# nkargas/Gen2-UHF-RFID-Reader

Measured on AMD Instinct MI355X. Metric: I/Q Msamples/s through matched_filter->gate->tag_decoder (+ EPC decodes/s), 40 kHz FM0, higher is better.
Workload: dtype f32; 1 GPU; configs[1]: batch of 1024 noise-replicas per GPU of the 71-round file_source_test stand-in trace, FM0 40 kHz BLF @ 2 Msps (1076066 raw I/Q samples each, sigma=0.002), generated and resident in HBM; streams_per_gpu=1024, hbm_bytes_traces=8815132672, parallelism=traces sharded per GPU, no collective

## Files before the change

### gen2-uhf-rfid-reader_amd/csrc/rfid_capi.hip

```cpp
#include <hip/hip_runtime.h>

#include <cmath>
#include <ctime>
#include <pthread.h>
#include <cstdio>
#include <cstdlib>
#include <cstring>
#include <deque>
#include <initializer_list>
#include <map>
#include <memory>
#include <new>
#include <vector>

#include "rfid_host_math.h"
#include "rfid_kernels.hpp"
#include "rfid_inventory.hpp"
#include "rfid_tracks.hpp"
#include "rfid_quality.hpp"
#include "rfid_mi355x.h"
#include "rfid_gen2_host.h"
#define LS2_LAUNCH(kernel, gx, gy, block, args) \
  hipLaunchKernelGGL(rfidk::kernel, dim3((unsigned)(gx), (unsigned)(gy)), dim3((unsigned)(block)), 0, ls2_stream, args)
static thread_local hipStream_t ls2_stream = nullptr;
static thread_local unsigned ls2_front_lds = 0;
#define LS2_LAUNCH_FRONT(kernel, gx, gy, block, args) \
  hipLaunchKernelGGL(rfidk::kernel, dim3((unsigned)(gx), (unsigned)(gy)), dim3((unsigned)(block)), ls2_front_lds, ls2_stream, args)
static double g_la_t[20] = {0};
static long g_la_n[20] = {0};
static bool g_la_on = false;
static inline void la_count(int k, double dt) { if (g_la_on) { g_la_t[k] += dt; g_la_n[k]++; } }
static inline double la_now() { struct timespec ts; clock_gettime(CLOCK_MONOTONIC, &ts); return 1e3 * (double)ts.tv_sec + 1e-6 * (double)ts.tv_nsec; }
struct LaTimer { int k; double t0; explicit LaTimer(int kk) : k(kk), t0(g_la_on ? la_now() : 0.0) {} ~LaTimer() { if (g_la_on) la_count(k, la_now() - t0); } };
#include "rfid_ls2_enqueue.hpp"

using namespace rfidk;

namespace {

struct DevBuf {
  void *p = nullptr;
  size_t cap = 0;
};

}

struct RfidKnobs {
  int long_stream = 1;
  int overlap = 1;
  int ls_calibrate = 1;
  int ls_debug = 0;
  int la_profile = 0;
  int front_unfused = 0;
  int front_chunks = 1;
  int fsm_lanes_min = -1;
  int dc_rounds = -1;
  int la_upload_kernel = 1;
  int front_lds_kb = -1;
  int inventory_slots = 0;
};

struct rfid_ctx {
  rfid_params prm;
  RfidKnobs knobs;
  int device = 0;
  hipStream_t stream = nullptr;
  char err[512];
  float t_cand[N_TCAND];

  rfid_reader_state rs;

  void *d_small = nullptr;
  GateState *d_gate1 = nullptr;
  int *d_io = nullptr;
  DevBuf s_in, s_out;
  DevBuf synth_tab;
  DevBuf ls2_ws;
  DevBuf ls2_ws_alt;
  bool ls2_mark_failed = false;
  bool y_touched = false;
  Ls2Ctl *ls2_host = nullptr;
  Ls2Ctl *d_ls2_ctl = nullptr;
  int ls2_P = 0;
  int ls2_rounds[3] = {0, 0, 0};
  bool ls2_generous = false;
  int ls_mode = 1;
  double ls_fixed_ms = 0.45, ls_ns_per_sample = 0.03, seq_ns_per_sample = 10.2;
  bool ls_calibrated = false;
  bool ls_measured = false;
  bool plan_for_stream = false;
  struct StreamIO {
    bool open = false;
    bool failed = false;
    bool ymode = false;
    int dec() const { return ymode ? 1 : DECIM; }
    int hist() const { return ymode ? 0 : 28; }
    int64_t max_chunk = 0, tail_max = 0;
    float2 *d_buf[2] = {nullptr, nullptr};
    rfid_cf32 *h_pin[2] = {nullptr, nullptr};
    hipStream_t copy_stream = nullptr;
    hipEvent_t ev_up[2] = {nullptr, nullptr};
    hipEvent_t ev_free[2] = {nullptr, nullptr};
    int cur = 0;
    bool pending = false;
    int pend_idx = 0;
    int64_t pend_new = 0;
    int64_t tail_len = 0;
    int64_t acc_new = 0;
    hipEvent_t ev_hist = nullptr;
    int64_t raw_base = 0;
    std::vector<rfid_stream_window> out_w;
    std::vector<rfid_decode_result> out_r;
    struct Pass {
      bool active = false;
// ... 77 lines not shown
  rfid_window *d_swin = nullptr;
  int *d_scount = nullptr;
  rfid_decode_result *d_sres = nullptr;
  rfid_scores *d_sscores = nullptr;
  static const int MF_HIST = NTAPS - 1 + DECIM - 1;
  rfid_cf32 mf_hist[MF_HIST];
  int64_t mf_seen = 0;

  int B = 0;
  int B_plan = 0;
  int64_t max_raw = 0, y_stride = 0;
  float2 *d_y = nullptr;
  float2 *y_view = nullptr;
  float2 *y() const { return y_view ? y_view : d_y; }
  GateState *d_gstate = nullptr;
  rfid_window *d_wtab = nullptr, *d_flat = nullptr;
  int wmax = 0, flat_cap = 0;
  int *d_wcount = nullptr, *d_flat_count = nullptr;
  int *d_ticket = nullptr;
  int ticket_flip = 0;
  rfid_decode_result *d_res = nullptr;
  int *d_sum = nullptr;
  const rfid_decode_result *sum_of = nullptr;
  rfid_scores *d_scores = nullptr;
  rfid_stream_stats *d_stats = nullptr;
  const int64_t *d_lens = nullptr;
  int64_t last_n_raw = 0;
  int decode_grid = 0;
  int n_cus = 256;
  hipEvent_t ev[5] = {nullptr, nullptr, nullptr, nullptr, nullptr};
  bool ev_valid[5] = {false, false, false, false, false};
  static const int MAX_CHUNKS = 16;
  hipStream_t stream2 = nullptr;
  hipEvent_t ev_mf[MAX_CHUNKS + 1], ev_gate[2 * MAX_CHUNKS], ev_pass = nullptr, ev_front_end = nullptr;
  struct ResultSet {
    float2 *d_y = nullptr;
    rfid_window *d_wtab = nullptr, *d_flat = nullptr;
    int *d_wcount = nullptr, *d_flat_count = nullptr;
    rfid_decode_result *d_res = nullptr;
    rfid_stream_stats *d_stats = nullptr;
  } alt;
  bool alt_have = false;
  void *plan_blk = nullptr, *alt_blk = nullptr;
  hipEvent_t ev_fe_done = nullptr, ev_tail_done[2] = {nullptr, nullptr};
  bool tail_recorded[2] = {false, false};
  int set_idx = 0;
  void *alt_y_blk = nullptr;
  hipEvent_t ev_y_free[2] = {nullptr, nullptr};
  bool y_recorded[2] = {false, false};
  int y_idx = 0;
  hipStream_t tail_stream = nullptr;
  struct Stage {
    void *blk = nullptr;
    hipEvent_t ev[2] = {nullptr, nullptr};
    bool enqueued = false;
  };
  struct Inventory : Stage {
    int max_tags = 0, slots = 0;
    rfid_tag_entry *d_ent = nullptr, *d_packed = nullptr;
    int *d_counts = nullptr, *d_over = nullptr, *d_off = nullptr, *d_head = nullptr;
    int n_streams = 0;
  } inv;
  struct Tracks : Stage {
    rfid_tag_read *d_reads = nullptr;
    int64_t cap = 0;
    int64_t *d_off = nullptr;
// ... 16 lines not shown
namespace {

void sio_free(rfid_ctx *c);
int sio_process(rfid_ctx *c, int b, int64_t n_new, bool flush);
int sio_submit(rfid_ctx *c, int b, int64_t n_new, bool flush);
int sio_collect(rfid_ctx *c);
void la_free(rfid_ctx *c);
int la_mf_work(rfid_ctx *c, const rfid_cf32 *in, int n_in, rfid_cf32 *out, int out_cap, int *n_produced);
int la_gate_work(rfid_ctx *c, const rfid_cf32 *in, int n_in, rfid_cf32 *out, int out_cap, int *n_consumed, int *n_written);
int la_gate_swallow(rfid_ctx *c, const rfid_cf32 *in, int n_in, rfid_cf32 *out, int out_cap, int *n_consumed, int *n_written);
bool la_decoder_result(rfid_ctx *c, const rfid_cf32 *in, int wlen, int type, rfid_decode_result *r);

int fail(rfid_ctx *c, int code, const char *what, hipError_t e = hipSuccess) {
  if (c) {
    if (e != hipSuccess)
      snprintf(c->err, sizeof(c->err), "%s: %s", what, hipGetErrorString(e));
    else
      snprintf(c->err, sizeof(c->err), "%s", what);
  }
  return code;
}

struct KnobEntry { const char *name, *env; int RfidKnobs::*field; int lo, hi; };
const KnobEntry g_knob_table[] = {
  {"long_stream", "RFID_LONG_STREAM", &RfidKnobs::long_stream, 0, 2},
  {"overlap", "RFID_OVERLAP", &RfidKnobs::overlap, 0, 2},
  {"ls_calibrate", "RFID_LS_CALIBRATE", &RfidKnobs::ls_calibrate, 0, 1},
  {"ls_debug", "RFID_LS_DEBUG", &RfidKnobs::ls_debug, 0, 1},
  {"la_profile", "RFID_LA_PROFILE", &RfidKnobs::la_profile, 0, 1},
  {"front_unfused", "RFID_FRONT_UNFUSED", &RfidKnobs::front_unfused, 0, 1},
  {"front_chunks", "RFID_FRONT_CHUNKS", &RfidKnobs::front_chunks, 1, rfid_ctx::MAX_CHUNKS},
  {"fsm_lanes_min", "RFID_LS2_FSM_LANES_MIN", &RfidKnobs::fsm_lanes_min, -1, 1 << 30},
  {"dc_rounds", "RFID_LS2_DC_ROUNDS", &RfidKnobs::dc_rounds, -1, 64},
  {"la_upload_kernel", "RFID_LA_UPLOAD_KERNEL", &RfidKnobs::la_upload_kernel, 0, 1},
  {"front_lds_kb", "RFID_LS_FRONT_LDS_KB", &RfidKnobs::front_lds_kb, -1, 64},
  {"inventory_slots", "RFID_INVENTORY_SLOTS", &RfidKnobs::inventory_slots, 0, 1024},
};
int clamp_int(long v, int lo, int hi) { return (int)(v < lo ? lo : (v > hi ? hi : v)); }
void knobs_from_env(RfidKnobs &k) {
  for (const KnobEntry &e : g_knob_table) {
    const char *v = getenv(e.env);
    if (!v || !*v) continue;
    char *end = nullptr;
    const long x = strtol(v, &end, 10);
    if (end == v) continue;
    k.*(e.field) = clamp_int(x, e.lo, e.hi);
  }
}

#define HIPCHK(c, call)                                                     \
  do {                                                                      \
    hipError_t e__ = (call);                                                \
    if (e__ != hipSuccess) return fail((c), RFID_ERR_HIP, #call, e__);      \
  } while (0)

#define HIPCHK_T(c, call)                                                   \
  do {                                                                      \
    hipError_t e__ = (call);                                                \
    if (e__ != hipSuccess) { (c)->y_touched = true; return fail((c), RFID_ERR_HIP, #call, e__); } \
  } while (0)

int grow(rfid_ctx *c, DevBuf &b, size_t bytes) {
  if (bytes <= b.cap) return RFID_OK;
  if (b.p) HIPCHK(c, hipFree(b.p));
  b.p = nullptr;
  b.cap = 0;
  size_t want = bytes < 4096 ? 4096 : bytes;
  HIPCHK(c, hipMalloc(&b.p, want));
// ... 179 lines not shown
    const double t_ls = c->ls_fixed_ms + 1e-6 * c->ls_ns_per_sample * (double)B * (double)n_dec;
    if (pass == 0 && !c->ls_calibrated && t_ls > 0.33 * t_seq && t_ls < 3.0 * t_seq) { ls_calibrate_lazily(c); continue; }
    return t_ls < 0.9 * t_seq;
  }
  return false;
}
bool ls_applicable(rfid_ctx *c, int B, int64_t n_dec) {
  if (c->ls_mode == 0 || B > 4096) return false;
  if (ls2_geometry(B, n_dec).P == 0) return false;
  return c->ls_mode == 2 || ls_pays_off(c, B, n_dec);
}
bool ls_may_apply(const rfid_ctx *c, int B, int64_t n_dec) {
  if (c->ls_mode == 0 || B > 4096) return false;
  if (ls2_geometry(B, n_dec).P == 0) return false;
  const double t_seq = 1e-6 * c->seq_ns_per_sample * (double)n_dec * (double)((B + 1023) / 1024);
  const double t_ls = c->ls_fixed_ms + 1e-6 * c->ls_ns_per_sample * (double)B * (double)n_dec;
  return c->ls_mode == 2 || t_ls < 3.0 * t_seq;
}
size_t ls_workspace_bytes(int B, int64_t n_dec, int64_t y_stride, int wmax) {
  const Ls2Geometry g = ls2_geometry(B, n_dec);
  return g.P ? ls2_layout(g, B, y_stride, wmax).total : 0;
}

int ls_calibrate(rfid_ctx *c);
void ls_note_last_pass(rfid_ctx *c);

struct LsOpts {
  bool carry = false;
  bool hold_last = false;
  bool force = false;
  bool ahead = false;
  const void *raw = nullptr; int64_t raw_stride = 0;
};
void ls_note_last_pass(rfid_ctx *c) {
  if (!c->d_ls2_ctl || !c->ls2_host) return;
  if (hipStreamQuery(c->stream) == hipSuccess) {
    const Ls2Ctl &k = *c->ls2_host;
    if (!c->ls2_generous && k.fail == 0 && k.ok == 0 && k.n_pieces > 0) c->ls2_generous = true;
  }
  (void)hipGetLastError();
}
int ls_enqueue(rfid_ctx *c, int64_t n_dec, const LsOpts &opt, int *enqueued) {
  *enqueued = 0;
  c->d_ls2_ctl = nullptr;
  const Ls2Geometry geo = ls2_geometry(c->B, n_dec);
  if (geo.P == 0 || c->B > 65535) return RFID_OK;
  const Ls2Layout L = ls2_layout(geo, c->B, c->y_stride, c->wmax);
  const bool ahead = opt.ahead && opt.raw && c->ls2_ws.cap >= L.total && c->ls2_ws_alt.cap >= L.total;
  if (opt.ahead && !ahead) return RFID_OK;
  if (L.total > c->ls2_ws.cap) {
    if (c->ls2_ws.p) { (void)hipFree(c->ls2_ws.p); c->ls2_ws.p = nullptr; c->ls2_ws.cap = 0; }
    if (hipMalloc(&c->ls2_ws.p, L.total) != hipSuccess) { (void)hipGetLastError(); c->ls2_ws.p = nullptr; return RFID_OK; }
    c->ls2_ws.cap = L.total;
  }
  if (!c->ls2_host) {
    if (hipHostMalloc((void **)&c->ls2_host, sizeof(Ls2Ctl) + 64, hipHostMallocDefault) != hipSuccess) {
      (void)hipGetLastError(); c->ls2_host = nullptr; return RFID_OK;
    }
    memset(c->ls2_host, 0, sizeof(Ls2Ctl) + 64);
  }
  Ls2Args a;
  memset(&a, 0, sizeof(a));
  a.y = c->y(); a.y_stride = c->y_stride; a.lens = c->d_lens; a.n_dec = n_dec; a.n_streams = c->B;
  if (ahead) std::swap(c->ls2_ws, c->ls2_ws_alt);
  ls2_bind(a, (char *)c->ls2_ws.p, L, geo);
  a.wtab = c->d_wtab; a.wmax = c->wmax; a.wcount = c->d_wcount; a.flat = c->d_flat; a.flat_count = c->d_flat_count; a.flat_cap = c->flat_cap;
  a.carry = opt.carry ? c->d_gstate : nullptr; a.carry_out = opt.carry ? c->d_gstate : nullptr;
  a.hold_last = opt.hold_last ? 1 : 0; a.force = opt.force ? 1 : 0;
  if (opt.raw) {
    a.fused = 1;
    a.raw = (const float2 *)opt.raw; a.raw_stride = opt.raw_stride;
    a.raw_vec_ok = ((opt.raw_stride & 1) == 0 && (((uintptr_t)opt.raw) & 15) == 0) ? 1 : 0;
    a.y_w = c->d_y;
  }
  ls2_stream = ahead ? c->stream2 : c->stream;
  {
    const int kb = (c->knobs.front_lds_kb >= 0) ? c->knobs.front_lds_kb : ((geo.NS >= 32768) ? 10 : 0);
    ls2_front_lds = (unsigned)kb * 1024u;
  }
  a.keep_flat_count = ahead ? 1 : 0;
  {
    static const int lanes_min_default = ls2_fsm_lanes_min();
    ls2_fsm_lanes_min() = (c->knobs.fsm_lanes_min >= 0) ? c->knobs.fsm_lanes_min : lanes_min_default;
  }
  auto mark = [](void *p, int pt) {
    rfid_ctx *cc = (rfid_ctx *)p;
    if (pt == 2) {
      if (ls2_stream == cc->stream2) {
        if (hipEventRecord(cc->ev_fe_done, cc->stream2) != hipSuccess || hipStreamWaitEvent(cc->stream, cc->ev_fe_done, 0) != hipSuccess ||
            hipMemsetAsync(cc->d_flat_count, 0, 2 * sizeof(int), cc->stream) != hipSuccess) cc->ls2_mark_failed = true;
        ls2_stream = cc->stream;
      }
      return;
    }
  };
  c->ls2_mark_failed = false;
  ls2_enqueue(a, true, c->ls2_rounds, c->ls2_generous, c->knobs.dc_rounds, ahead ? +mark : nullptr, c);
  ls2_stream = c->stream;
  HIPCHK(c, hipGetLastError());
  if (c->ls2_mark_failed) return fail(c, RFID_ERR_HIP, "long-stream front end: stream hand-over");
  HIPCHK(c, hipMemcpyAsync(c->ls2_host, a.ctl, sizeof(Ls2Ctl) + sizeof(int), hipMemcpyDeviceToHost, c->stream));
  c->d_ls2_ctl = a.ctl;
  c->ls2_P = geo.P;
  *enqueued = 1;
  if (c->knobs.ls_debug) {
    HIPCHK(c, hipStreamSynchronize(c->stream));
    const Ls2Ctl &k = *c->ls2_host;
    fprintf(stderr, "[ls2] pieces %d P %d fail %d ok %d | avg:", k.n_pieces, geo.P, k.fail, k.ok);
    for (int r = 0; r <= c->ls2_rounds[0]; ++r) fprintf(stderr, " %d/%d", k.avg_count[r], k.avg_list[r]);
    fprintf(stderr, " | fsm:");
    for (int r = 0; r <= c->ls2_rounds[1]; ++r) fprintf(stderr, " %d", k.fsm_count[r]);
    fprintf(stderr, " | dc:");
    for (int r = 0; r <= c->ls2_rounds[2]; ++r) fprintf(stderr, " %d", k.dc_count[r]);
    fprintf(stderr, " | units %d windows %d\n", k.n_units, k.n_windows);
    std::vector<Ls2AvgRun> ar((size_t)geo.NS);
    std::vector<int> aT((size_t)geo.NS);
    std::vector<Ls2Piece> pc((size_t)geo.NS);
    HIPCHK(c, hipMemcpy(ar.data(), a.arun, sizeof(Ls2AvgRun) * ar.size(), hipMemcpyDeviceToHost));
    HIPCHK(c, hipMemcpy(aT.data(), a.aT, sizeof(int) * aT.size(), hipMemcpyDeviceToHost));
    HIPCHK(c, hipMemcpy(pc.data(), a.piece, sizeof(Ls2Piece) * pc.size(), hipMemcpyDeviceToHost));
    long hist_m[8] = {0}, hist_d[8] = {0};
    int shown = 0;
    {
      long hist_len[6] = {0}; int max_len = 0; long n_wide = 0, n_over = 0;
      for (int i = 0; i < geo.NS; ++i) {
        const int len = pc[(size_t)i].len;
        if (len <= 0) continue;
        if (len > max_len) max_len = len;
        const int q = (int)(4.0 * len / geo.P);
        hist_len[q < 2 ? 0 : (q < 4 ? 1 : (q < 6 ? 2 : (q < 8 ? 3 : (q < 16 ? 4 : 5))))]++;
        if (ar[(size_t)i].wide & 2) n_wide++;
        if (ar[(size_t)i].wide & 4) n_over++;
      }
      fprintf(stderr, "[ls2] piece lengths in P (< 0.5, < 1, < 1.5, < 2, < 4, more): %ld %ld %ld %ld %ld %ld, longest %d; last run wide: %ld, exact end put in: %ld\n",
// ... 72 lines not shown
    return RFID_OK;
  }
  hipEvent_t e0 = nullptr, e1 = nullptr;
  bool ok = hipEventCreate(&e0) == hipSuccess && hipEventCreate(&e1) == hipSuccess;
  double t_seq[2] = {0, 0}, t_ls[2] = {0, 0};
  for (int k = 0; k < 2 && ok; ++k) {
    int64_t n = 0;
    const int B = k ? B_big : 1;
    ok = rfid_synth_gen2(c, &p, slots.data(), k ? n_big : n_big / 4, d_base, stride, 0.0f, 77u, 0, &n) == RFID_OK && n == L[k];
    ok = ok && rfid_synth_replicas(c, d_base, L[k], d_many, stride, B, 0.003f, 78u, 0) == RFID_OK;
    ok = ok && rfid_batch_plan(c, B, L[k]) == RFID_OK;
    for (int mode = 0; mode <= 2 && ok; mode += 2) {
      c->ls_mode = mode;
      float best = 1e30f;
      for (int rep = 0; rep < 3 && ok; ++rep) {
        ok = hipEventRecord(e0, c->stream) == hipSuccess && rfid_batch_process(c, d_many, stride, L[k], nullptr, 0) == RFID_OK &&
             hipEventRecord(e1, c->stream) == hipSuccess && hipStreamSynchronize(c->stream) == hipSuccess;
        float ms = 0.0f;
        ok = ok && hipEventElapsedTime(&ms, e0, e1) == hipSuccess;
        if (rep > 0 && ms < best) best = ms;
      }
      if (mode == 2 && ok) ok = c->d_ls2_ctl != nullptr && c->ls2_host->ok != 0;
      (mode ? t_ls : t_seq)[k] = best;
    }
  }
  c->ls_mode = saved_mode;
  if (e0) (void)hipEventDestroy(e0);
  if (e1) (void)hipEventDestroy(e1);
  (void)hipStreamSynchronize(c->stream);
  (void)hipFree(d_base);
  (void)hipFree(d_many);
  free_plan(c);
  c->d_ls2_ctl = nullptr;
  if (!ok) { (void)hipGetLastError(); return RFID_OK; }
  const double n0 = (double)(L[0] / DECIM), n1 = (double)(L[1] / DECIM), N1 = n1 * B_big;
  const double slope = (t_ls[1] - t_ls[0]) / (N1 - n0);
  const double fixed = t_ls[0] - slope * n0;
  if (slope > 0.0 && fixed > 0.0 && t_seq[1] > 0.0) {
    c->ls_ns_per_sample = 1.25 * slope * 1e6;
    c->ls_fixed_ms = fixed;
    c->seq_ns_per_sample = t_seq[1] / n1 * 1e6;
    c->ls_measured = true;
  }
  c->ls_calibrated = true;
  if (c->knobs.ls_debug)
    fprintf(stderr, "[ls2] calibration: fused %.3f / %.3f ms, long-stream %.3f / %.3f ms for 1 x %.0f / %d x %.0f samples -> %.2f ns/sample of the longest trace vs %.3f ms + %.4f ns/sample of all\n",
            t_seq[0], t_seq[1], t_ls[0], t_ls[1], n0, B_big, n1, c->seq_ns_per_sample, c->ls_fixed_ms, c->ls_ns_per_sample);
  return RFID_OK;
}

struct LsCalCache { bool done = false, ok = false; double fixed_ms = 0, ns_all = 0, ns_seq = 0; };
LsCalCache g_ls_cal[64];
pthread_mutex_t g_ls_cal_mu = PTHREAD_MUTEX_INITIALIZER;
void ls_calibrate_lazily(rfid_ctx *c) {
  c->ls_calibrated = true;
  if (!c->knobs.ls_calibrate || c->device < 0 || c->device >= 64) return;
  pthread_mutex_lock(&g_ls_cal_mu);
  LsCalCache &k = g_ls_cal[c->device];
  if (!k.done) {
    k.done = true;
    rfid_ctx *t = nullptr;
    if (rfid_ctx_create(&c->prm, c->device, &t) == RFID_OK && t) {
      t->ls_calibrated = true;
      t->ls_mode = 1;
      if (ls_calibrate(t) == RFID_OK && t->ls_measured) {
        k.ok = true; k.fixed_ms = t->ls_fixed_ms; k.ns_all = t->ls_ns_per_sample; k.ns_seq = t->seq_ns_per_sample;
// ... 51 lines not shown
    pthread_mutex_lock(&prop_mu);
    if (!dev_info[device].known) {
      hipDeviceProp_t prop;
      if (hipGetDeviceProperties(&prop, device) == hipSuccess) {
        dev_info[device].known = true;
        dev_info[device].gfx950 = strncmp(prop.gcnArchName, "gfx950", 6) == 0;
        dev_info[device].cus = prop.multiProcessorCount;
      }
    }
    is_gfx950 = dev_info[device].known && dev_info[device].gfx950;
    pthread_mutex_unlock(&prop_mu);
  }
  if (!is_gfx950) return RFID_ERR_NO_DEVICE;
  rfid_ctx *c = new (std::nothrow) rfid_ctx();
  if (c) c->n_cus = dev_info[device].cus;
  if (!c) return RFID_ERR_CAPACITY;
  c->prm = *p;
  c->device = device;
  c->err[0] = 0;
  compute_t_cand(c->t_cand, p->sample_rate);
  knobs_from_env(c->knobs);
  if (c->knobs.la_profile) g_la_on = true;
  c->ls_mode = c->knobs.long_stream;
  init_reader_state(c);
  memset(c->mf_hist, 0, sizeof(c->mf_hist));
  int rc = RFID_OK;
  do {
    if (hipSetDevice(device) != hipSuccess) { rc = RFID_ERR_NO_DEVICE; break; }
    if (hipStreamCreateWithFlags(&c->stream, hipStreamNonBlocking) != hipSuccess) { rc = RFID_ERR_HIP; break; }
    for (int i = 0; i < 5; ++i)
      if (hipEventCreate(&c->ev[i]) != hipSuccess) { rc = RFID_ERR_HIP; break; }
    if (rc) break;
    if (hipStreamCreateWithFlags(&c->stream2, hipStreamNonBlocking) != hipSuccess) { rc = RFID_ERR_HIP; break; }
    for (int i = 0; i <= rfid_ctx::MAX_CHUNKS; ++i) c->ev_mf[i] = nullptr;
    for (int i = 0; i < 2 * rfid_ctx::MAX_CHUNKS; ++i) c->ev_gate[i] = nullptr;
    if (!rc && (hipEventCreate(&c->ev_pass) != hipSuccess || hipEventCreate(&c->ev_front_end) != hipSuccess ||
                hipEventCreateWithFlags(&c->ev_fe_done, hipEventDisableTiming) != hipSuccess ||
                hipEventCreateWithFlags(&c->ev_tail_done[0], hipEventDisableTiming) != hipSuccess ||
                hipEventCreateWithFlags(&c->ev_tail_done[1], hipEventDisableTiming) != hipSuccess ||
                hipEventCreateWithFlags(&c->ev_y_free[0], hipEventDisableTiming) != hipSuccess ||
                hipEventCreateWithFlags(&c->ev_y_free[1], hipEventDisableTiming) != hipSuccess))
      rc = RFID_ERR_HIP;
    if (rc) break;
    {
      char *blk = nullptr;
      const size_t slot = 256, n_slots = 4 + 1 + 1 + 1 + 1 + 1 + 1;
      if (hipMalloc((void **)&blk, slot * n_slots) != hipSuccess || hipMemset(blk, 0, slot * n_slots) != hipSuccess) { rc = RFID_ERR_HIP; c->d_small = blk; break; }
      static_assert(sizeof(GateState) <= 4 * 256 && sizeof(rfid_scores) <= 256 && sizeof(rfid_decode_result) <= 256, "slots");
      c->d_small = blk;
      c->d_gate1 = (GateState *)blk;
      c->d_io = (int *)(blk + 4 * slot);
      c->d_swin = (rfid_window *)(blk + 5 * slot);
      c->d_scount = (int *)(blk + 6 * slot);
      c->d_ticket = (int *)(blk + 7 * slot);
      c->d_sres = (rfid_decode_result *)(blk + 8 * slot);
      c->d_sscores = (rfid_scores *)(blk + 9 * slot);
    }
  } while (0);
  if (rc != RFID_OK) { rfid_ctx_destroy(c); return rc; }
  *out = c;
  return RFID_OK;
}

int rfid_ctx_destroy(rfid_ctx *c) {
  if (!c) return RFID_ERR_INVALID;
  if (c->knobs.la_profile && (g_la_n[0] || g_la_n[1]))
    fprintf(stderr, "[la] mf_work %ld calls %.2f ms (upload queued %.2f, the call's filter enqueued %.2f, wait for its outputs %.2f, passes submitted from here %.2f) | "
            "gate_work %ld calls %.2f ms | decoder_work %ld calls %.2f ms | reader_work_tx %ld calls %.2f ms | lookahead_enable %.2f ms | "
            "%ld passes: collected %.2f ms (waiting for the device %.2f, fetching windows %.2f), submitted %.2f ms (the pass's filter %.2f, front end's launch list %.2f, "
            "decoder %.2f, packet of results %.2f)\n",
            g_la_n[0], g_la_t[0], g_la_t[4], g_la_t[5], g_la_t[8], g_la_t[6], g_la_n[1], g_la_t[1], g_la_n[2], g_la_t[2], g_la_n[3], g_la_t[3], g_la_t[9],
            g_la_n[10], g_la_t[10], g_la_t[7], g_la_t[12], g_la_t[11], g_la_t[14], g_la_t[13], g_la_t[15], g_la_t[16]);
  (void)hipSetDevice(c->device);
  if (c->stream) (void)hipStreamSynchronize(c->stream);
  la_free(c);
  sio_free(c);
  free_plan(c);
  void *ptrs[] = {c->d_small, c->s_in.p, c->s_out.p, c->synth_tab.p, c->ls2_ws.p, c->ls2_ws_alt.p};
  for (void *p : ptrs)
    if (p) (void)hipFree(p);
  if (c->ls2_host) (void)hipHostFree(c->ls2_host);
  for (int i = 0; i < 5; ++i)
    if (c->ev[i]) (void)hipEventDestroy(c->ev[i]);
  for (rfid_ctx::Stage *st : {(rfid_ctx::Stage *)&c->inv, (rfid_ctx::Stage *)&c->trk, (rfid_ctx::Stage *)&c->qual})
    for (int i = 0; i < 2; ++i)
      if (st->ev[i]) (void)hipEventDestroy(st->ev[i]);
  if (c->stream2) {
    (void)hipStreamSynchronize(c->stream2);
    for (int i = 0; i <= rfid_ctx::MAX_CHUNKS; ++i)
      if (c->ev_mf[i]) (void)hipEventDestroy(c->ev_mf[i]);
    for (int i = 0; i < 2 * rfid_ctx::MAX_CHUNKS; ++i)
      if (c->ev_gate[i]) (void)hipEventDestroy(c->ev_gate[i]);
    if (c->ev_pass) (void)hipEventDestroy(c->ev_pass);
    if (c->ev_front_end) (void)hipEventDestroy(c->ev_front_end);
    if (c->ev_fe_done) (void)hipEventDestroy(c->ev_fe_done);
    for (int i = 0; i < 2; ++i) {
      if (c->ev_tail_done[i]) (void)hipEventDestroy(c->ev_tail_done[i]);
      if (c->ev_y_free[i]) (void)hipEventDestroy(c->ev_y_free[i]);
    }
    (void)hipStreamDestroy(c->stream2);
  }
  if (c->stream) (void)hipStreamDestroy(c->stream);
  delete c;
  return RFID_OK;
}

int rfid_ctx_reset(rfid_ctx *c) {
  if (!c) return RFID_ERR_INVALID;
  HIPCHK(c, hipSetDevice(c->device));
  init_reader_state(c);
  memset(c->mf_hist, 0, sizeof(c->mf_hist));
  c->mf_seen = 0;
  if (c->la.on) { la_free(c); sio_free(c); }
  HIPCHK(c, hipMemsetAsync(c->d_gate1, 0, sizeof(GateState), c->stream));
  HIPCHK(c, hipStreamSynchronize(c->stream));
  return RFID_OK;
}

void *rfid_ctx_stream(rfid_ctx *c) { return c ? (void *)c->stream : nullptr; }

int rfid_get_state(const rfid_ctx *c, rfid_reader_state *out) {
  if (!c || !out) return RFID_ERR_INVALID;
  *out = c->rs;
  return RFID_OK;
}

int rfid_print_results(const rfid_ctx *c, char *buf, int cap, int *len) {
  if (!c || !buf || cap <= 0) return RFID_ERR_INVALID;
  const rfid_reader_state &rs = c->rs;
  int n = 0;
  n += snprintf(buf + n, cap - n, "\n --------------------------\n");
  n += snprintf(buf + n, cap - n, "| Number of queries/queryreps sent : %d\n", rs.n_queries_sent - 1);
  n += snprintf(buf + n, cap - n, "| Current Inventory round : %d\n", rs.cur_inventory_round);
  n += snprintf(buf + n, cap - n, " --------------------------\n");
// ... 155 lines not shown
    e = hipMemset(c->d_wcount, 0, sz_c + sz_fc);
  }
  if (e != hipSuccess) {
    (void)hipGetLastError();
    free_plan(c);
    return fail(c, RFID_ERR_HIP, "rfid_batch_plan: workspace allocation", e);
  }
  c->B = c->B_plan = n_streams;
  if (wide_traces(c)) {
    if (hipMalloc((void **)&c->d_sum, sizeof(int) * ((size_t)c->flat_cap + 4)) != hipSuccess) { (void)hipGetLastError(); c->d_sum = nullptr; }
  }
  {
    const size_t need = sizeof(float2) * (size_t)c->y_stride * n_streams + (sizeof(rfid_window) * 3 + sizeof(rfid_decode_result)) * (size_t)c->flat_cap +
                        sizeof(rfid_stream_stats) * (size_t)n_streams;
    size_t free_b = 0, total_b = 0;
    if (c->knobs.overlap >= 2 && n_streams >= 64 && hipMemGetInfo(&free_b, &total_b) == hipSuccess && need < free_b / 8) {
      hipError_t e2 = hipMalloc(&c->alt_blk, sz_set);
      if (e2 == hipSuccess) {
        bind_set((char *)c->alt_blk, c->alt.d_y, c->alt.d_wtab, c->alt.d_flat, c->alt.d_wcount, c->alt.d_flat_count, c->alt.d_res, c->alt.d_stats);
        e2 = hipMemset(c->alt.d_wcount, 0, sz_c + sz_fc);
      }
      if (e2 == hipSuccess) c->alt_have = true;
      else {
        (void)hipGetLastError();
        if (c->alt_blk) (void)hipFree(c->alt_blk);
        c->alt_blk = nullptr;
        c->alt = rfid_ctx::ResultSet();
      }
    }
  }
  if (ls_may_apply(c, n_streams, n_dec)) {
    {
      size_t free_b = 0, total_b = 0;
      if (!c->alt_have && !c->plan_for_stream && c->knobs.overlap != 0 && sz_y >= ((size_t)16 << 20) && hipMemGetInfo(&free_b, &total_b) == hipSuccess && sz_y < free_b / 8) {
        if (hipMalloc(&c->alt_y_blk, sz_y) == hipSuccess) c->alt.d_y = (float2 *)c->alt_y_blk;
        else { (void)hipGetLastError(); c->alt_y_blk = nullptr; }
      }
    }
    const size_t need = ls_workspace_bytes(n_streams, n_dec, c->y_stride, c->wmax);
    if (need > c->ls2_ws.cap) {
      if (c->ls2_ws.p) (void)hipFree(c->ls2_ws.p);
      c->ls2_ws.p = nullptr; c->ls2_ws.cap = 0;
      if (hipMalloc(&c->ls2_ws.p, need) == hipSuccess) c->ls2_ws.cap = need;
      else { (void)hipGetLastError(); c->ls2_ws.p = nullptr; }
    }
    if (c->alt.d_y && !c->alt_have && (c->knobs.overlap != 0) && c->ls2_ws.p && need > c->ls2_ws_alt.cap) {
      size_t free_b = 0, total_b = 0;
      if (c->ls2_ws_alt.p) (void)hipFree(c->ls2_ws_alt.p);
      c->ls2_ws_alt.p = nullptr; c->ls2_ws_alt.cap = 0;
      if (hipMemGetInfo(&free_b, &total_b) == hipSuccess && need < free_b / 8) {
        if (hipMalloc(&c->ls2_ws_alt.p, need) == hipSuccess) c->ls2_ws_alt.cap = need;
        else { (void)hipGetLastError(); c->ls2_ws_alt.p = nullptr; }
      }
    }
  }
  c->decode_grid = c->n_cus * 8;
  for (int i = 0; i < 5; ++i) c->ev_valid[i] = false;
  return RFID_OK;
}

int rfid_batch_set_streams(rfid_ctx *c, int n_streams) {
  if (!c || n_streams <= 0) return RFID_ERR_INVALID;
  if (!c->B_plan) return RFID_ERR_STATE;
  if (n_streams > c->B_plan) return RFID_ERR_CAPACITY;
  c->B = n_streams;
  return RFID_OK;
}
// ... 330 lines not shown
  *n = nrows;
  if (nrows > cap) return fail(c, RFID_ERR_CAPACITY, "rfid_batch_get_window_quality: cap is smaller than the number of EPC windows");
  const int64_t take = (cap < q.rows) ? cap : q.rows;
  if (take > 0) {
    HIPCHK(c, hipMemcpyAsync(out, q.d_table + (size_t)stream * (size_t)q.rows, sizeof(rfid_read_quality) * (size_t)take, hipMemcpyDeviceToHost, c->stream));
    HIPCHK(c, hipStreamSynchronize(c->stream));
  }
  return RFID_OK;
}

int rfid_batch_quality_ms(rfid_ctx *c, float *ms) {
  if (!c || !ms) return RFID_ERR_INVALID;
  return stage_ms(c, c->qual, ms);
}

int rfid_batch_process(rfid_ctx *c, const void *d_raw, int64_t raw_stride, int64_t n_raw, const void *d_lens,
                       int want_scores) {
  if (!c || !d_raw || n_raw < 0 || raw_stride < n_raw) return RFID_ERR_INVALID;
  if (!c->B) return RFID_ERR_STATE;
  if (n_raw > c->max_raw) return RFID_ERR_CAPACITY;
  ls_note_last_pass(c);
  const int64_t n_out = n_raw / DECIM;
  const int64_t tiles = (n_out + MF_TILE - 1) / MF_TILE;
  const int nch = c->knobs.front_chunks;
  if (nch < 2 && ls_applicable(c, c->B, n_out)) {
    HIPCHK(c, hipSetDevice(c->device));
    { int rj = join_tails(c); if (rj) return rj; }
    int rc;
    if (raw_stride >= 2) {
      c->d_lens = (const int64_t *)d_lens;
      c->last_n_raw = n_raw;
      c->n_chunks_last = 0;
      const bool ahead = c->alt.d_y != nullptr && c->ls2_ws_alt.p != nullptr && !c->alt_have && (c->knobs.overlap != 0);
      if (ahead) {
        std::swap(c->d_y, c->alt.d_y);
        c->y_idx ^= 1;
        if (c->y_touched) {
          HIPCHK_T(c, hipEventRecord(c->ev_pass, c->stream));
          HIPCHK_T(c, hipStreamWaitEvent(c->stream2, c->ev_pass, 0));
          c->y_touched = false;
        }
        if (c->y_recorded[c->y_idx]) {
          HIPCHK_T(c, hipStreamWaitEvent(c->stream2, c->ev_y_free[c->y_idx], 0));
          c->y_recorded[c->y_idx] = false;
        }
      }
      HIPCHK_T(c, hipEventRecord(c->ev[0], c->stream));
      HIPCHK_T(c, hipEventRecord(c->ev[1], c->stream));
      c->ev_valid[0] = c->ev_valid[1] = true;
      int enq = 0;
      LsOpts lo;
      lo.raw = d_raw; lo.raw_stride = raw_stride; lo.ahead = ahead;
      if ((rc = ls_enqueue(c, n_out, lo, &enq))) { c->y_touched = true; return rc; }
      if (!enq && ahead) {
        std::swap(c->d_y, c->alt.d_y); c->y_idx ^= 1;
        c->y_touched = true;
        lo.ahead = false;
        if ((rc = ls_enqueue(c, n_out, lo, &enq))) { c->y_touched = true; return rc; }
      }
      const bool ahead_now = ahead && lo.ahead;
      if (enq) {
        c->fused_last = 2;
        MfFallbackArgs f;
        f.m.x = (const float2 *)d_raw; f.m.x_stride = raw_stride; f.m.n_raw = n_raw; f.m.lens = c->d_lens;
        f.m.n_out = n_out; f.m.in_off = -(NTAPS - 1);
        f.m.vec_ok = ((raw_stride & 1) == 0 && (((uintptr_t)d_raw) & 15) == 0) ? 1 : 0;
        f.m.y = c->d_y; f.m.y_stride = c->y_stride; f.m.tile0 = 0; f.m.stream0 = 0;
        f.skip_if = &c->d_ls2_ctl->ok; f.n_tiles = tiles;
        const int64_t gx = (tiles < 4096) ? tiles : 4096;
        for (int s0 = 0; s0 < c->B && gx > 0; s0 += 65535) {
          f.m.stream0 = s0;
          const int ns = (c->B - s0 < 65535) ? (c->B - s0) : 65535;
          hipLaunchKernelGGL(mf_fallback_kernel, dim3((unsigned)gx, (unsigned)ns), dim3(MF_THREADS), 0, c->stream, f);
          HIPCHK_T(c, hipGetLastError());
        }
        if ((rc = rfid_batch_gate_impl(c, &c->d_ls2_ctl->ok)) || (rc = rfid_batch_decode(c, want_scores)) || (rc = rfid_batch_stats(c))) { c->y_touched = true; return rc; }
        if (ahead_now) {
          HIPCHK_T(c, hipEventRecord(c->ev_y_free[c->y_idx], c->stream));
          c->y_recorded[c->y_idx] = true;
        } else {
          c->y_touched = true;
        }
        return RFID_OK;
      }
    }
    c->y_touched = true;
    if ((rc = batch_mf_on(c, c->stream, d_raw, raw_stride, n_raw, d_lens))) return rc;
    int enq = 0;
    LsOpts lo;
    if ((rc = ls_enqueue(c, n_out, lo, &enq))) return rc;
// ... 142 lines not shown
int rfid_ctx_get_knob(const rfid_ctx *c, const char *name, int *value) {
  if (!c || !name || !value) return RFID_ERR_INVALID;
  for (const KnobEntry &e : g_knob_table)
    if (strcmp(name, e.name) == 0) { *value = (e.field == &RfidKnobs::long_stream) ? c->ls_mode : c->knobs.*(e.field); return RFID_OK; }
  return RFID_ERR_INVALID;
}

int rfid_batch_ls_report(const rfid_ctx *c, rfid_ls_report *out) {
  if (!c || !out) return RFID_ERR_INVALID;
  memset(out, 0, sizeof(*out));
  if (!c->d_ls2_ctl || !c->ls2_host) return RFID_OK;
  (void)hipSetDevice(c->device);
  if (hipStreamSynchronize(c->stream) != hipSuccess) return RFID_ERR_HIP;
  const Ls2Ctl &k = *c->ls2_host;
  const int ra = c->ls2_rounds[0], rf = c->ls2_rounds[1], rd = c->ls2_rounds[2];
  out->pieces = k.n_pieces;
  out->units = k.n_units;
  out->chunk = c->ls2_P;
  out->avg_rounds = k.avg_rounds; out->avg_reruns = k.avg_reruns;
  out->fsm_rounds = k.fsm_rounds;
  out->dc_rounds = k.dc_rounds; out->dc_reruns = k.dc_reruns;
  for (int r = 0; r <= rf; ++r) out->cuts_dropped += k.fsm_count[r];
  out->windows = k.n_windows;
  out->dc_finished = k.dc_finished;
  out->verified = (k.ok != 0) ? 1 : 0;
  out->gave_up = out->verified ? 0 : (k.fail ? k.fail : (k.avg_count[ra] ? 2 : (k.fsm_count[rf] ? 3 : (k.dc_count[rd] ? 4 : 5))));
  return RFID_OK;
}

int rfid_batch_sync(rfid_ctx *c) {
  if (!c) return RFID_ERR_INVALID;
  HIPCHK(c, hipSetDevice(c->device));
  HIPCHK(c, hipStreamSynchronize(c->stream2));
  HIPCHK(c, hipStreamSynchronize(c->stream));
  return RFID_OK;
}

int rfid_batch_timing_get(rfid_ctx *c, rfid_batch_timing *out) {
  if (!c || !out) return RFID_ERR_INVALID;
  HIPCHK(c, hipSetDevice(c->device));
  HIPCHK(c, hipStreamSynchronize(c->stream2));
  HIPCHK(c, hipStreamSynchronize(c->stream));
  float ms[4] = {0, 0, 0, 0};
  float front = 0.0f;
  if (c->n_chunks_last > 0) {
    for (int k = 0; k < c->n_chunks_last; ++k) {
      float t = 0.0f;
      HIPCHK(c, hipEventElapsedTime(&t, c->ev_mf[k], c->ev_mf[k + 1]));
      ms[0] += t;
      HIPCHK(c, hipEventElapsedTime(&t, c->ev_gate[2 * k], c->ev_gate[2 * k + 1]));
      ms[1] += t;
    }
    HIPCHK(c, hipEventElapsedTime(&front, c->ev_mf[0], c->ev_front_end));
    for (int i = 2; i < 4; ++i)
      if (c->ev_valid[i] && c->ev_valid[i + 1]) HIPCHK(c, hipEventElapsedTime(&ms[i], c->ev[i], c->ev[i + 1]));
    out->total_ms = front + ms[2] + ms[3];
  } else {
    for (int i = 0; i < 4; ++i)
      if (c->ev_valid[i] && c->ev_valid[i + 1]) HIPCHK(c, hipEventElapsedTime(&ms[i], c->ev[i], c->ev[i + 1]));
    out->total_ms = ms[0] + ms[1] + ms[2] + ms[3];
  }
  out->mf_ms = ms[0]; out->gate_ms = ms[1]; out->decode_ms = ms[2]; out->stats_ms = ms[3];
  out->front_ms = (c->n_chunks_last > 0) ? front : (ms[0] + ms[1]);
  out->front_chunks = (c->n_chunks_last > 0) ? c->n_chunks_last : 1;
  out->decode_launches = 1;
  out->fused_front = c->fused_last;
  out->reserved_ = 0;
  return RFID_OK;
}

int rfid_batch_get_stats(rfid_ctx *c, rfid_stream_stats *out, int n_streams) {
  if (!c || !out || n_streams <= 0) return RFID_ERR_INVALID;
  if (!c->B) return RFID_ERR_STATE;
  if (n_streams > c->B) n_streams = c->B;
// ... 513 lines not shown
```

### gen2-uhf-rfid-reader_amd/csrc/rfid_ls2_enqueue.hpp

```cpp
#pragma once
#include <stddef.h>
#ifndef LS2_FIN_WPB
#define LS2_FIN_WPB 1
#endif
#ifndef LS2_LAUNCH_FRONT
#define LS2_LAUNCH_FRONT LS2_LAUNCH
#endif
#include <stdint.h>

namespace rfidk {

constexpr int LS2_TARGET_PIECES = 131072;
constexpr int LS2_MIN_PIECE = 512;

struct Ls2Geometry {
  int P = 0, max_b = 0, NS = 0;
  int Pc = 0, max_bc = 0;
  int64_t vstride = 0, cstride = 0, wb_stride = 0;
  int n1 = 0, n2 = 0;
};
inline Ls2Geometry ls2_geometry(int n_streams, int64_t n_dec, int min_piece = LS2_MIN_PIECE, int target = LS2_TARGET_PIECES) {
  Ls2Geometry g;
  if (n_streams <= 0 || n_dec < 2 * (int64_t)LS2_FINE * min_piece) return g;
  int64_t P = ((int64_t)n_streams * n_dec + target - 1) / target;
// ... 154 lines not shown
  } else {
    LS2_LAUNCH(ls2_pieces_kernel, (NS + 255) / 256, 1, 256, a);
  }
  auto rerun_grid = [&](int round, int most) { const int g = (round == 1) ? most : most / 2; return (NS < g) ? NS : g; };
  auto chain_g = [](int slots) { const int per = ls2_chain_slots(); int g = (slots + per - 1) / per; return g < 1 ? 1 : (g > LS2_CHAIN_GMAX ? LS2_CHAIN_GMAX : g); };
  const int g_avg = chain_g(a.max_b), g_seq = chain_g(a.max_bc);
  if (!fused) LS2_LAUNCH(ls2_avg_first_kernel, 8 * ((NS + 7) / 8), 1, 64, a);
  a.chain_g = g_avg; a.stamp++;
  LS2_LAUNCH(ls2_avg_chain_kernel, g_avg, B, LS2_CHAIN_THREADS, a);
  for (int r = 1; r <= a.avg_rounds; ++r) {
    a.round = r;
    LS2_LAUNCH(ls2_avg_rerun_kernel, rerun_grid(r, 32768), 1, 64, a);
    a.stamp++;
    LS2_LAUNCH(ls2_avg_chain_kernel, g_avg, B, LS2_CHAIN_THREADS, a);
  }
  for (int r = 0; r <= a.fsm_rounds; ++r) {
    a.round = r;
    if (NH >= ls2_fsm_lanes_min()) LS2_LAUNCH(ls2_fsm_lanes_kernel, (NH + LS2_FSM_LANES - 1) / LS2_FSM_LANES, 1, 64, U(a));
    else LS2_LAUNCH(ls2_fsm_kernel, NH, 1, 64, U(a));
    LS2_LAUNCH(ls2_fsm_chain_kernel, (NH + 255) / 256, 1, 256, U(a));
  }
  {
    const int N1 = B * a.dcb_n1, N2 = B * a.dcb_n2;
    for (int r = 0; r <= a.dc_rounds; ++r) {
      a.round = r;
      LS2_LAUNCH(ls2_dcb_run_kernel, (r <= 3 || NH < 4096) ? NH : 4096, 1, 64, U(a));
      LS2_LAUNCH(ls2_dcb_up1_kernel, N1, 1, 64, U(a));
      if (a.dcb_top == 2) LS2_LAUNCH(ls2_dcb_up2_kernel, N2, 1, 64, U(a));
      LS2_LAUNCH(ls2_dcb_top_kernel, B, 1, 64, U(a));
      if (a.dcb_top == 2) LS2_LAUNCH(ls2_dcb_down2_kernel, N2, 1, 64, U(a));
      LS2_LAUNCH(ls2_dcb_down1_kernel, N1, 1, 64, U(a));
    }
    a.round = 0;
    {
      LS2_LAUNCH(ls2_dcb_incr_kernel, NH, 1, 64, U(a));
      LS2_LAUNCH(ls2_dcb_finish_kernel<LS2_FIN_WPB>, ls2_fin_waves(B) / LS2_FIN_WPB, B, 64 * LS2_FIN_WPB, U(a));
    }
  }
  a.round = 0;
  a.stamp++;
  a.chain_g = g_seq;
  LS2_LAUNCH(ls2_seq_kernel, g_seq, B, LS2_CHAIN_THREADS, U(a));
  LS2_LAUNCH(ls2_assemble_kernel, NH, 1, 64, U(a));
  if (a.carry_out) LS2_LAUNCH(ls2_carry_kernel, B, 1, 64, U(a));
  if (rounds_out) { rounds_out[0] = a.avg_rounds; rounds_out[1] = a.fsm_rounds; rounds_out[2] = a.dc_rounds; }
}
#endif

}
```

Baseline: 394,900 Msamples/s.

## Add optional second lane stream and multi-slot host control buffers for long-stream overlap

```diff
diff --git a/gen2-uhf-rfid-reader_amd/csrc/rfid_capi.hip b/gen2-uhf-rfid-reader_amd/csrc/rfid_capi.hip
--- a/gen2-uhf-rfid-reader_amd/csrc/rfid_capi.hip
+++ b/gen2-uhf-rfid-reader_amd/csrc/rfid_capi.hip
@@ -55,8 +55,10 @@
   int front_chunks = 1;
   int fsm_lanes_min = -1;
   int dc_rounds = -1;
+  int ls2_alt_min_kb = 16384;
   int la_upload_kernel = 1;
   int front_lds_kb = -1;
+  int ls2_lanes = 1;
   int inventory_slots = 0;
 };
 
@@ -80,6 +82,12 @@
   bool ls2_mark_failed = false;
   bool y_touched = false;
   Ls2Ctl *ls2_host = nullptr;
+  static const int LS2_HOST_SLOTS = 4;
+  static const size_t LS2_HOST_STRIDE = (sizeof(Ls2Ctl) + 64 + 255) & ~(size_t)255;
+  char *ls2_host_blk = nullptr;
+  hipEvent_t ev_ctl[LS2_HOST_SLOTS] = {nullptr, nullptr, nullptr, nullptr};
+  bool ctl_pending[LS2_HOST_SLOTS] = {false, false, false, false};
+  int ctl_slot = 0;
   Ls2Ctl *d_ls2_ctl = nullptr;
   int ls2_P = 0;
   int ls2_rounds[3] = {0, 0, 0};
@@ -223,6 +231,8 @@
   bool ev_valid[5] = {false, false, false, false, false};
   static const int MAX_CHUNKS = 16;
   hipStream_t stream2 = nullptr;
+  hipStream_t stream3 = nullptr;
+  hipEvent_t ev_lane_done[2] = {nullptr, nullptr};
   hipEvent_t ev_mf[MAX_CHUNKS + 1], ev_gate[2 * MAX_CHUNKS], ev_pass = nullptr, ev_front_end = nullptr;
   struct ResultSet {
     float2 *d_y = nullptr;
@@ -305,8 +315,10 @@
   {"front_chunks", "RFID_FRONT_CHUNKS", &RfidKnobs::front_chunks, 1, rfid_ctx::MAX_CHUNKS},
   {"fsm_lanes_min", "RFID_LS2_FSM_LANES_MIN", &RfidKnobs::fsm_lanes_min, -1, 1 << 30},
   {"dc_rounds", "RFID_LS2_DC_ROUNDS", &RfidKnobs::dc_rounds, -1, 64},
+  {"ls2_alt_min_kb", "RFID_LS2_ALT_MIN_KB", &RfidKnobs::ls2_alt_min_kb, 0, 1 << 30},
   {"la_upload_kernel", "RFID_LA_UPLOAD_KERNEL", &RfidKnobs::la_upload_kernel, 0, 1},
   {"front_lds_kb", "RFID_LS_FRONT_LDS_KB", &RfidKnobs::front_lds_kb, -1, 64},
+  {"ls2_lanes", "RFID_LS2_LANES", &RfidKnobs::ls2_lanes, 1, 2},
   {"inventory_slots", "RFID_INVENTORY_SLOTS", &RfidKnobs::inventory_slots, 0, 1024},
 };
 int clamp_int(long v, int lo, int hi) { return (int)(v < lo ? lo : (v > hi ? hi : v)); }
@@ -552,14 +564,23 @@
   bool ahead = false;
   const void *raw = nullptr; int64_t raw_stride = 0;
 };
+void ls_note_slot(rfid_ctx *c, int i) {
+  const Ls2Ctl &k = *(const Ls2Ctl *)(c->ls2_host_blk + (size_t)i * rfid_ctx::LS2_HOST_STRIDE);
+  if (!c->ls2_generous && k.fail == 0 && k.ok == 0 && k.n_pieces > 0) c->ls2_generous = true;
+  c->ctl_pending[i] = false;
+}
 void ls_note_last_pass(rfid_ctx *c) {
-  if (!c->d_ls2_ctl || !c->ls2_host) return;
+  if (!c->ls2_host_blk) return;
+  bool any = false;
+  for (int i = 0; i < rfid_ctx::LS2_HOST_SLOTS; ++i) any = any || c->ctl_pending[i];
+  if (!any) return;
   if (hipStreamQuery(c->stream) == hipSuccess) {
-    const Ls2Ctl &k = *c->ls2_host;
-    if (!c->ls2_generous && k.fail == 0 && k.ok == 0 && k.n_pieces > 0) c->ls2_generous = true;
+    for (int i = 0; i < rfid_ctx::LS2_HOST_SLOTS; ++i)
+      if (c->ctl_pending[i]) ls_note_slot(c, i);
   }
   (void)hipGetLastError();
 }
+hipStream_t ls2_lane_stream(const rfid_ctx *c) { return (c->knobs.ls2_lanes >= 2 && c->y_idx == 1) ? c->stream3 : c->stream2; }
 int ls_enqueue(rfid_ctx *c, int64_t n_dec, const LsOpts &opt, int *enqueued) {
   *enqueued = 0;
   c->d_ls2_ctl = nullptr;
@@ -573,11 +594,18 @@
     if (hipMalloc(&c->ls2_ws.p, L.total) != hipSuccess) { (void)hipGetLastError(); c->ls2_ws.p = nullptr; return RFID_OK; }
     c->ls2_ws.cap = L.total;
   }
-  if (!c->ls2_host) {
-    if (hipHostMalloc((void **)&c->ls2_host, sizeof(Ls2Ctl) + 64, hipHostMallocDefault) != hipSuccess) {
-      (void)hipGetLastError(); c->ls2_host = nullptr; return RFID_OK;
-    }
-    memset(c->ls2_host, 0, sizeof(Ls2Ctl) + 64);
+  if (!c->ls2_host_blk) {
+    const size_t bytes = rfid_ctx::LS2_HOST_STRIDE * rfid_ctx::LS2_HOST_SLOTS;
+    if (hipHostMalloc((void **)&c->ls2_host_blk, bytes, hipHostMallocDefault) != hipSuccess) {
+      (void)hipGetLastError(); c->ls2_host_blk = nullptr; return RFID_OK;
+    }
+    memset(c->ls2_host_blk, 0, bytes);
+    c->ls2_host = (Ls2Ctl *)c->ls2_host_blk;
+  }
+  const int ctl_slot = c->ctl_slot;
+  if (c->ctl_pending[ctl_slot]) {
+    HIPCHK(c, hipEventSynchronize(c->ev_ctl[ctl_slot]));
+    ls_note_slot(c, ctl_slot);
   }
   Ls2Args a;
   memset(&a, 0, sizeof(a));
@@ -593,7 +621,7 @@
     a.raw_vec_ok = ((opt.raw_stride & 1) == 0 && (((uintptr_t)opt.raw) & 15) == 0) ? 1 : 0;
     a.y_w = c->d_y;
   }
-  ls2_stream = ahead ? c->stream2 : c->stream;
+  ls2_stream = ahead ? ls2_lane_stream(c) : c->stream;
   {
     const int kb = (c->knobs.front_lds_kb >= 0) ? c->knobs.front_lds_kb : ((geo.NS >= 32768) ? 10 : 0);
     ls2_front_lds = (unsigned)kb * 1024u;
@@ -605,13 +633,11 @@
   }
   auto mark = [](void *p, int pt) {
     rfid_ctx *cc = (rfid_ctx *)p;
-    if (pt == 2) {
-      if (ls2_stream == cc->stream2) {
-        if (hipEventRecord(cc->ev_fe_done, cc->stream2) != hipSuccess || hipStreamWaitEvent(cc->stream, cc->ev_fe_done, 0) != hipSuccess ||
-            hipMemsetAsync(cc->d_flat_count, 0, 2 * sizeof(int), cc->stream) != hipSuccess) cc->ls2_mark_failed = true;
-        ls2_stream = cc->stream;
-      }
-      return;
+    if (pt == (cc->knobs.ls2_lanes >= 2 ? 3 : 2) && ls2_stream != cc->stream) {
+      hipEvent_t done = cc->ev_lane_done[ls2_stream == cc->stream3 ? 1 : 0];
+      if (hipEventRecord(done, ls2_stream) != hipSuccess || hipStreamWaitEvent(cc->stream, done, 0) != hipSuccess ||
+          hipMemsetAsync(cc->d_flat_count, 0, 2 * sizeof(int), cc->stream) != hipSuccess) cc->ls2_mark_failed = true;
+      ls2_stream = cc->stream;
     }
   };
   c->ls2_mark_failed = false;
@@ -619,7 +645,11 @@
   ls2_stream = c->stream;
   HIPCHK(c, hipGetLastError());
   if (c->ls2_mark_failed) return fail(c, RFID_ERR_HIP, "long-stream front end: stream hand-over");
+  c->ls2_host = (Ls2Ctl *)(c->ls2_host_blk + (size_t)ctl_slot * rfid_ctx::LS2_HOST_STRIDE);
   HIPCHK(c, hipMemcpyAsync(c->ls2_host, a.ctl, sizeof(Ls2Ctl) + sizeof(int), hipMemcpyDeviceToHost, c->stream));
+  HIPCHK(c, hipEventRecord(c->ev_ctl[ctl_slot], c->stream));
+  c->ctl_pending[ctl_slot] = true;
+  c->ctl_slot = (ctl_slot + 1) % rfid_ctx::LS2_HOST_SLOTS;
   c->d_ls2_ctl = a.ctl;
   c->ls2_P = geo.P;
   *enqueued = 1;
@@ -758,6 +788,7 @@
   (void)hipFree(d_many);
   free_plan(c);
   c->d_ls2_ctl = nullptr;
+  for (bool &pending : c->ctl_pending) pending = false;
   if (!ok) { (void)hipGetLastError(); return RFID_OK; }
   const double n0 = (double)(L[0] / DECIM), n1 = (double)(L[1] / DECIM), N1 = n1 * B_big;
   const double slope = (t_ls[1] - t_ls[0]) / (N1 - n0);
@@ -875,6 +906,7 @@
       if (hipEventCreate(&c->ev[i]) != hipSuccess) { rc = RFID_ERR_HIP; break; }
     if (rc) break;
     if (hipStreamCreateWithFlags(&c->stream2, hipStreamNonBlocking) != hipSuccess) { rc = RFID_ERR_HIP; break; }
+    if (hipStreamCreateWithFlags(&c->stream3, hipStreamNonBlocking) != hipSuccess) { rc = RFID_ERR_HIP; break; }
     for (int i = 0; i <= rfid_ctx::MAX_CHUNKS; ++i) c->ev_mf[i] = nullptr;
     for (int i = 0; i < 2 * rfid_ctx::MAX_CHUNKS; ++i) c->ev_gate[i] = nullptr;
     if (!rc && (hipEventCreate(&c->ev_pass) != hipSuccess || hipEventCreate(&c->ev_front_end) != hipSuccess ||
@@ -884,6 +916,10 @@
                 hipEventCreateWithFlags(&c->ev_y_free[0], hipEventDisableTiming) != hipSuccess ||
                 hipEventCreateWithFlags(&c->ev_y_free[1], hipEventDisableTiming) != hipSuccess))
       rc = RFID_ERR_HIP;
+    for (int i = 0; i < 2 && !rc; ++i)
+      if (hipEventCreateWithFlags(&c->ev_lane_done[i], hipEventDisableTiming) != hipSuccess) rc = RFID_ERR_HIP;
+    for (int i = 0; i < rfid_ctx::LS2_HOST_SLOTS && !rc; ++i)
+      if (hipEventCreateWithFlags(&c->ev_ctl[i], hipEventDisableTiming) != hipSuccess) rc = RFID_ERR_HIP;
     if (rc) break;
     {
       char *blk = nullptr;
@@ -915,6 +951,7 @@
             g_la_n[0], g_la_t[0], g_la_t[4], g_la_t[5], g_la_t[8], g_la_t[6], g_la_n[1], g_la_t[1], g_la_n[2], g_la_t[2], g_la_n[3], g_la_t[3], g_la_t[9],
             g_la_n[10], g_la_t[10], g_la_t[7], g_la_t[12], g_la_t[11], g_la_t[14], g_la_t[13], g_la_t[15], g_la_t[16]);
   (void)hipSetDevice(c->device);
+  if (c->stream3) (void)hipStreamSynchronize(c->stream3);
   if (c->stream) (void)hipStreamSynchronize(c->stream);
   la_free(c);
   sio_free(c);
@@ -922,7 +959,11 @@
   void *ptrs[] = {c->d_small, c->s_in.p, c->s_out.p, c->synth_tab.p, c->ls2_ws.p, c->ls2_ws_alt.p};
   for (void *p : ptrs)
     if (p) (void)hipFree(p);
-  if (c->ls2_host) (void)hipHostFree(c->ls2_host);
+  if (c->ls2_host_blk) (void)hipHostFree(c->ls2_host_blk);
+  for (int i = 0; i < rfid_ctx::LS2_HOST_SLOTS; ++i)
+    if (c->ev_ctl[i]) (void)hipEventDestroy(c->ev_ctl[i]);
+  for (int i = 0; i < 2; ++i)
+    if (c->ev_lane_done[i]) (void)hipEventDestroy(c->ev_lane_done[i]);
   for (int i = 0; i < 5; ++i)
     if (c->ev[i]) (void)hipEventDestroy(c->ev[i]);
   for (rfid_ctx::Stage *st : {(rfid_ctx::Stage *)&c->inv, (rfid_ctx::Stage *)&c->trk, (rfid_ctx::Stage *)&c->qual})
@@ -943,6 +984,7 @@
     }
     (void)hipStreamDestroy(c->stream2);
   }
+  if (c->stream3) (void)hipStreamDestroy(c->stream3);
   if (c->stream) (void)hipStreamDestroy(c->stream);
   delete c;
   return RFID_OK;
@@ -1164,7 +1206,7 @@
   if (ls_may_apply(c, n_streams, n_dec)) {
     {
       size_t free_b = 0, total_b = 0;
-      if (!c->alt_have && !c->plan_for_stream && c->knobs.overlap != 0 && sz_y >= ((size_t)16 << 20) && hipMemGetInfo(&free_b, &total_b) == hipSuccess && sz_y < free_b / 8) {
+      if (!c->alt_have && !c->plan_for_stream && c->knobs.overlap != 0 && sz_y >= ((size_t)c->knobs.ls2_alt_min_kb << 10) && hipMemGetInfo(&free_b, &total_b) == hipSuccess && sz_y < free_b / 8) {
         if (hipMalloc(&c->alt_y_blk, sz_y) == hipSuccess) c->alt.d_y = (float2 *)c->alt_y_blk;
         else { (void)hipGetLastError(); c->alt_y_blk = nullptr; }
       }
@@ -1561,21 +1603,24 @@
       c->last_n_raw = n_raw;
       c->n_chunks_last = 0;
       const bool ahead = c->alt.d_y != nullptr && c->ls2_ws_alt.p != nullptr && !c->alt_have && (c->knobs.overlap != 0);
+      hipStream_t lane = c->stream;
       if (ahead) {
         std::swap(c->d_y, c->alt.d_y);
         c->y_idx ^= 1;
+        lane = ls2_lane_stream(c);
         if (c->y_touched) {
           HIPCHK_T(c, hipEventRecord(c->ev_pass, c->stream));
-          HIPCHK_T(c, hipStreamWaitEvent(c->stream2, c->ev_pass, 0));
+          HIPCHK_T(c, hipStreamWaitEvent(lane, c->ev_pass, 0));
           c->y_touched = false;
         }
         if (c->y_recorded[c->y_idx]) {
-          HIPCHK_T(c, hipStreamWaitEvent(c->stream2, c->ev_y_free[c->y_idx], 0));
+          HIPCHK_T(c, hipStreamWaitEvent(lane, c->ev_y_free[c->y_idx], 0));
           c->y_recorded[c->y_idx] = false;
         }
       }
-      HIPCHK_T(c, hipEventRecord(c->ev[0], c->stream));
-      HIPCHK_T(c, hipEventRecord(c->ev[1], c->stream));
+      hipStream_t ev_stream = (ahead && c->knobs.ls2_lanes >= 2) ? lane : c->stream;
+      HIPCHK_T(c, hipEventRecord(c->ev[0], ev_stream));
+      HIPCHK_T(c, hipEventRecord(c->ev[1], ev_stream));
       c->ev_valid[0] = c->ev_valid[1] = true;
       int enq = 0;
       LsOpts lo;
@@ -1585,6 +1630,10 @@
         std::swap(c->d_y, c->alt.d_y); c->y_idx ^= 1;
         c->y_touched = true;
         lo.ahead = false;
+        if (ev_stream != c->stream) {
+          HIPCHK_T(c, hipEventRecord(c->ev[0], c->stream));
+          HIPCHK_T(c, hipEventRecord(c->ev[1], c->stream));
+        }
         if ((rc = ls_enqueue(c, n_out, lo, &enq))) { c->y_touched = true; return rc; }
       }
       const bool ahead_now = ahead && lo.ahead;
@@ -1793,6 +1842,7 @@
   if (!c) return RFID_ERR_INVALID;
   HIPCHK(c, hipSetDevice(c->device));
   HIPCHK(c, hipStreamSynchronize(c->stream2));
+  HIPCHK(c, hipStreamSynchronize(c->stream3));
   HIPCHK(c, hipStreamSynchronize(c->stream));
   return RFID_OK;
 }
@@ -1801,6 +1851,7 @@
   if (!c || !out) return RFID_ERR_INVALID;
   HIPCHK(c, hipSetDevice(c->device));
   HIPCHK(c, hipStreamSynchronize(c->stream2));
+  HIPCHK(c, hipStreamSynchronize(c->stream3));
   HIPCHK(c, hipStreamSynchronize(c->stream));
   float ms[4] = {0, 0, 0, 0};
   float front = 0.0f;
diff --git a/gen2-uhf-rfid-reader_amd/csrc/rfid_ls2_enqueue.hpp b/gen2-uhf-rfid-reader_amd/csrc/rfid_ls2_enqueue.hpp
--- a/gen2-uhf-rfid-reader_amd/csrc/rfid_ls2_enqueue.hpp
+++ b/gen2-uhf-rfid-reader_amd/csrc/rfid_ls2_enqueue.hpp
@@ -210,6 +210,7 @@
       LS2_LAUNCH(ls2_dcb_down1_kernel, N1, 1, 64, U(a));
     }
     a.round = 0;
+    if (mark) mark(mark_arg, 3);
     {
       LS2_LAUNCH(ls2_dcb_incr_kernel, NH, 1, 64, U(a));
       LS2_LAUNCH(ls2_dcb_finish_kernel<LS2_FIN_WPB>, ls2_fin_waves(B) / LS2_FIN_WPB, B, 64 * LS2_FIN_WPB, U(a));
```

New measurement: 394,800 Msamples/s (median of 2 runs). No clear change (-0.0%).
